# status-im/nim-blscurve

Hardware: AMD Instinct MI355X
Metric: BLS sig verifications/sec (batch) (higher is better)
Workload: dtype int64

## Files before the change

nim-blscurve_amd/csrc/kernels.hip:

```cpp
#include <hip/hip_runtime.h>

#include <algorithm>
#include <atomic>
#include <chrono>
#include <cstdio>
#include <cstdlib>
#include <cstring>
#include <mutex>
#include <string>
#include <unordered_map>
#include <vector>

#include "../../include/blscurve_mi355x.h"
#include "deser.hpp"
#include "h2c.hpp"
#include "pairing.hpp"
#include "vereach.hpp"
#include "aggsets.hpp"
#include "combsets.hpp"
#include "c12.hpp"
#include "teamvm.hpp"
#include "rowfp.hpp"
#include "rowvm.hpp"
#include "plan.hpp"
// ... 1519 lines not shown
    return g2_aff{fp2{ld_fp_int(w), ld_fp_int(w + FPW)}, fp2{ld_fp_int(w + 2 * FPW), ld_fp_int(w + 3 * FPW)}};
}
__device__ __forceinline__ g1_jac soa_ld_jac(const uint4* b, size_t stride, size_t i, const g1_jac*) { return soa_ld_g1(b, stride, i); }
__device__ __forceinline__ g2_jac soa_ld_jac(const uint4* b, size_t stride, size_t i, const g2_jac*) { return soa_ld_g2(b, stride, i); }
__device__ __forceinline__ void soa_st_jac(uint4* b, size_t stride, size_t i, const g1_jac& a) { soa_st_g1(b, stride, i, a); }
__device__ __forceinline__ void soa_st_jac(uint4* b, size_t stride, size_t i, const g2_jac& a) { soa_st_g2(b, stride, i, a); }
__device__ __forceinline__ g1_jac ld_jac_int(const uint32_t* w, const g1_jac*) { return ld_g1_int(w); }
__device__ __forceinline__ g2_jac ld_jac_int(const uint32_t* w, const g2_jac*) { return ld_g2_int(w); }
__device__ __forceinline__ void st_jac_int(uint32_t* w, const g1_jac& a) { st_g1_int(w, a); }
__device__ __forceinline__ void st_jac_int(uint32_t* w, const g2_jac& a) { st_g2_int(w, a); }
__device__ __forceinline__ void st_jac_blst(uint32_t* w, const g1_jac& a) { st_g1_blst(w, a); }
__device__ __forceinline__ void st_jac_blst(uint32_t* w, const g2_jac& a) { st_g2_blst(w, a); }
template <class F> struct fld;
template <> struct fld<fp> { static constexpr int W = FPW; static constexpr int AFFB = 96; };
template <> struct fld<fp2> { static constexpr int W = 2 * FPW; static constexpr int AFFB = 192; };
__device__ __forceinline__ g1_jac padd(const g1_jac& a, const g1_jac& b) { return jac_add_body(a, b); }
__device__ __forceinline__ g2_jac padd(const g2_jac& a, const g2_jac& b) { return jac_add(a, b); }

template <class F>
__global__ void __launch_bounds__(WAVE) k_pip_convert(const uint8_t* __restrict__ pts, uint32_t n, uint32_t* __restrict__ pts_int) {
    uint32_t i = blockIdx.x * WAVE + threadIdx.x;
    if (i >= n) return;
    aff<F> q = ld_aff_blst(reinterpret_cast<const uint32_t*>(pts + (size_t)i * fld<F>::AFFB), (const aff<F>*)nullptr);
    uint32_t* o = pts_int + (size_t)i * 2 * fld<F>::W;
    st_aff_int(o, q);
    o[FP_N] = aff_is_inf(q) ? 1u : 0u;
}
#if defined(__HIP_DEVICE_COMPILE__)
#include "../build/msm_asm.inc"
__device__ __forceinline__ uint32_t msm_bucket_asm(const uint32_t* pts, const uint32_t* srt, uint32_t cnt, uint4* buckets, uint32_t ostride16, uint32_t off16) {
    uint32_t flag;
    const uint64_t a = (uint64_t)(uintptr_t)srt;
    asm volatile(BLS_MSM_ASM_BODY : "=v"(flag) : "s"(pts), "v"((uint32_t)a), "v"((uint32_t)(a >> 32)), "v"(cnt), "s"(buckets), "s"(ostride16), "v"(off16) : BLS_MSM_ASM_CLOBBERS);
    return flag;
}
#endif
template <class F>
__global__ void __launch_bounds__(WAVE, sizeof(F) == sizeof(fp) ? 2 : 1) k_pip_bucket(const uint32_t* __restrict__ pts, const uint32_t* __restrict__ sorted, const uint32_t* __restrict__ offs,
                                                     const uint32_t* __restrict__ hist, const uint32_t* __restrict__ order, uint32_t n, uint32_t cbk,
                                                     uint32_t total, uint32_t g0, uint32_t gcount, uint4* __restrict__ buckets) {
    uint32_t t = blockIdx.x * WAVE + threadIdx.x;
    if (t >= gcount) return;
    uint32_t g = g0 + (order ? order[g0 + t] : t);
    uint32_t w = g >> cbk, cnt = hist[g], off = offs[g];
    const uint32_t* srt = sorted + (size_t)w * n + off;
#if defined(__HIP_DEVICE_COMPILE__)
    if constexpr (sizeof(F) == sizeof(fp)) {
        if (!msm_bucket_asm(pts, srt, cnt, buckets, total * 16u, g * 16u)) return;
    }
#endif
    xyzz<F> acc = xyzz_inf<F>();
    if (cnt) {
        uint32_t e = srt[0];
        const uint32_t* pw = pts + (size_t)(e & 0x7fffffffu) * (2 * fld<F>::W);
        aff<F> q = ld_aff_int(pw, (const aff<F>*)nullptr);
        if (e >> 31) q.y = f_neg(q.y);
        F one_or_zero = f_select(pw[FP_N] != 0, f_zero<F>(), f_one<F>());
        acc = xyzz<F>{q.x, q.y, one_or_zero, one_or_zero};
    }
    for (uint32_t j = 1; j < cnt; j++) {
        uint32_t e = srt[j];
        const uint32_t* pw = pts + (size_t)(e & 0x7fffffffu) * (2 * fld<F>::W);
        aff<F> q = ld_aff_int(pw, (const aff<F>*)nullptr);
        if (e >> 31) q.y = f_neg(q.y);
        acc = xyzz_add_aff_flag(acc, q, pw[FP_N] != 0);
    }
    soa_st_jac(buckets, total, g, jac_from_xyzz(acc));
}
template <class F>
__global__ void __launch_bounds__(WAVE) k_pip_segred(const uint4* __restrict__ buckets, uint32_t total, uint32_t cbk, uint32_t L, uint32_t nseg_total,
                                                     uint32_t t0, uint32_t tcount, uint4* __restrict__ segout) {
    uint32_t t = blockIdx.x * WAVE + threadIdx.x;
    if (t >= tcount) return;
    t += t0;
    uint32_t segs_per_win = (1u << cbk) / L;
    uint32_t w = t / segs_per_win, b0 = (t % segs_per_win) * L;
    jac<F> S = jac_inf<F>(), T = jac_inf<F>();
    for (uint32_t j = L; j-- > 0;) {
        jac<F> B = soa_ld_jac(buckets, total, ((size_t)w << cbk) | (b0 + j), (const jac<F>*)nullptr);
        S = padd(S, B);
        T = padd(T, S);
    }
    jac<F> acc = jac_inf<F>();
#pragma clang loop unroll(disable)
    for (int i = (int)cbk - 1; i >= 0; i--) {
        acc = jac_dbl(acc);
        if ((b0 >> i) & 1) acc = padd(acc, S);
    }
    acc = padd(acc, T);
    soa_st_jac(segout, nseg_total, t, acc);
}
template <int T>
struct team_quad_fp {
    uint32_t h;
    template <int J>
    __device__ __forceinline__ fp from(const fp& x) const {
        if (T == 4) return fp_quad_perm<J * 0x55>(x);
        return fp_quad_perm<(J ? 0xf5 : 0xa0)>(x);
    }
    __device__ __forceinline__ fp pick4(const fp& a0, const fp& a1, const fp& a2, const fp& a3) const {
        return fp_select((h & 1) != 0, fp_select((h & 2) != 0, a3, a1), fp_select((h & 2) != 0, a2, a0));
    }
    __device__ __forceinline__ void mul4(fp& r0, fp& r1, fp& r2, fp& r3, const fp& a0, const fp& b0, const fp& a1, const fp& b1, const fp& a2, const fp& b2, const fp& a3, const fp& b3) const {
        if (T == 4) {
            fp x = fp_mul(pick4(a0, a1, a2, a3), pick4(b0, b1, b2, b3));
            r0 = from<0>(x); r1 = from<1>(x); r2 = from<2>(x); r3 = from<3>(x);
        } else {
            const bool o = h != 0;
            fp x = fp_mul(fp_select(o, a1, a0), fp_select(o, b1, b0));
            fp y = fp_mul(fp_select(o, a3, a2), fp_select(o, b3, b2));
            r0 = from<0>(x); r1 = from<1>(x); r2 = from<0>(y); r3 = from<1>(y);
        }
    }
    __device__ __forceinline__ void mul3(fp& r0, fp& r1, fp& r2, const fp& a0, const fp& b0, const fp& a1, const fp& b1, const fp& a2, const fp& b2) const {
        fp r3;
        mul4(r0, r1, r2, r3, a0, b0, a1, b1, a2, b2, a2, b2);
    }
    __device__ __forceinline__ void sqr3(fp& r0, fp& r1, fp& r2, const fp& a0, const fp& a1, const fp& a2) const {
        if (T == 4) {
            fp x = fp_sqr(pick4(a0, a1, a2, a2));
            r0 = from<0>(x); r1 = from<1>(x); r2 = from<2>(x);
        } else {
            const bool o = h != 0;
            fp x = fp_sqr(fp_select(o, a1, a0));
            fp y = fp_sqr(a2);
            r0 = from<0>(x); r1 = from<1>(x); r2 = y;
        }
    }
    __device__ __forceinline__ void mul2(fp& r0, fp& r1, const fp& a0, const fp& b0, const fp& a1, const fp& b1) const {
        const bool o = (h & 1) != 0;
        fp x = fp_mul(fp_select(o, a1, a0), fp_select(o, b1, b0));
        if (T == 4) { r0 = fp_quad_perm<0xa0>(x); r1 = fp_quad_perm<0xf5>(x); }
        else { r0 = from<0>(x); r1 = from<1>(x); }
    }
    __device__ __forceinline__ void sqr2(fp& r0, fp& r1, const fp& a0, const fp& a1) const {
        const bool o = (h & 1) != 0;
        fp x = fp_sqr(fp_select(o, a1, a0));
        if (T == 4) { r0 = fp_quad_perm<0xa0>(x); r1 = fp_quad_perm<0xf5>(x); }
        else { r0 = from<0>(x); r1 = from<1>(x); }
    }
    __device__ __forceinline__ fp mul1(const fp& a, const fp& b) const { return fp_mul(a, b); }
};
template <int T>
__global__ void __launch_bounds__(WAVE) k_pip_segred_team(const uint4* __restrict__ buckets, uint32_t total, uint32_t cbk, uint32_t L, uint32_t nseg_total,
                                                          uint32_t t0, uint32_t tcount, uint4* __restrict__ segout) {
    uint32_t lane = blockIdx.x * WAVE + threadIdx.x, t = lane / T;
    if (t >= tcount) return;
    t += t0;
    const team_quad_fp<T> team{threadIdx.x & (T - 1)};
    uint32_t segs_per_win = (1u << cbk) / L;
    uint32_t w = t / segs_per_win, b0 = (t % segs_per_win) * L;
    g1_jac S = jac_inf<fp>(), Tt = jac_inf<fp>();
#pragma clang loop unroll(disable)
    for (uint32_t j = L; j-- > 0;) {
        g1_jac B = soa_ld_g1(buckets, total, ((size_t)w << cbk) | (b0 + j));
        S = jac_add_team(S, B, team);
        Tt = jac_add_team(Tt, S, team);
    }
    g1_jac acc = jac_inf<fp>();
#pragma clang loop unroll(disable)
    for (int i = (int)cbk - 1; i >= 0; i--) {
        acc = jac_dbl_team(acc, team);
        if ((b0 >> i) & 1) acc = jac_add_team(acc, S, team);
    }
    acc = jac_add_team(acc, Tt, team);
    if ((threadIdx.x & (T - 1)) == 0) soa_st_g1(segout, nseg_total, t, acc);
}
template <class F>
__global__ void __launch_bounds__(WAVE) k_pip_winpart(const uint4* __restrict__ segout, uint32_t nseg_total, uint32_t segs_per_win, uint32_t w0, uint32_t* __restrict__ part) {
    uint32_t w = w0 + blockIdx.x, sp = blockIdx.y, nsplit = gridDim.y;
    jac<F> acc = jac_inf<F>();
    for (uint32_t j = sp * WAVE + threadIdx.x; j < segs_per_win; j += WAVE * nsplit)
        acc = padd(acc, soa_ld_jac(segout, nseg_total, (size_t)w * segs_per_win + j, (const jac<F>*)nullptr));
    for (int d = 32; d >= 1; d >>= 1) {
        jac<F> o = shfl_down_struct(acc, d);
        acc = padd(acc, o);
    }
    if (threadIdx.x == 0) st_jac_int(part + ((size_t)w * nsplit + sp) * (3 * fld<F>::W), acc);
}
__device__ __forceinline__ fp fp_bcast(const fp& a, int src) {
    fp r;
#pragma unroll
    for (int i = 0; i < FP_N; i++) r.l[i] = __shfl(a.l[i], src, WAVE);
    return r;
}
struct team_wave_fp {
    __device__ __forceinline__ void mul3(fp& r0, fp& r1, fp& r2, const fp& a0, const fp& b0, const fp& a1, const fp& b1, const fp& a2, const fp& b2) const {
        const uint32_t l = threadIdx.x;
        fp r = fp_mul(fp_select(l == 0, a0, fp_select(l == 1, a1, a2)), fp_select(l == 0, b0, fp_select(l == 1, b1, b2)));
        r0 = fp_bcast(r, 0); r1 = fp_bcast(r, 1); r2 = fp_bcast(r, 2);
    }
    __device__ __forceinline__ void sqr3(fp& r0, fp& r1, fp& r2, const fp& a0, const fp& a1, const fp& a2) const {
        const uint32_t l = threadIdx.x;
        fp r = fp_sqr(fp_select(l == 0, a0, fp_select(l == 1, a1, a2)));
        r0 = fp_bcast(r, 0); r1 = fp_bcast(r, 1); r2 = fp_bcast(r, 2);
    }
    __device__ __forceinline__ fp mul1(const fp& a, const fp& b) const { return fp_mul(a, b); }
};
__device__ __forceinline__ g1_jac g1_dbl_coop(const g1_jac& p) { return jac_dbl_team(p, team_quad_fp<4>{threadIdx.x & 3u}); }
__device__ __forceinline__ g1_jac dbl_coop(const g1_jac& p) { return g1_dbl_coop(p); }
__device__ __forceinline__ g2_jac dbl_coop(const g2_jac& p) { return g2_dbl_coop(p, threadIdx.x & ~7u, threadIdx.x & 7u); }
__device__ __forceinline__ g1_jac bcast0(const g1_jac& a) { return g1_jac{fp_bcast(a.x, 0), fp_bcast(a.y, 0), fp_bcast(a.z, 0)}; }
__device__ __forceinline__ g2_jac bcast0(const g2_jac& a) {
    return g2_jac{fp2{fp_bcast(a.x.c0, 0), fp_bcast(a.x.c1, 0)}, fp2{fp_bcast(a.y.c0, 0), fp_bcast(a.y.c1, 0)}, fp2{fp_bcast(a.z.c0, 0), fp_bcast(a.z.c1, 0)}};
}
template <class F>
__global__ void __launch_bounds__(WAVE) k_pip_winsum(const uint32_t* __restrict__ part, uint32_t nsplit, pip_win W, uint32_t w0, uint32_t* __restrict__ winout) {
    uint32_t w = w0 + blockIdx.x;
    jac<F> acc = jac_inf<F>();
    for (uint32_t j = threadIdx.x; j < nsplit; j += WAVE) acc = padd(acc, ld_jac_int(part + ((size_t)w * nsplit + j) * (3 * fld<F>::W), (const jac<F>*)nullptr));
    int top = 32;
    while (top >= 1 && (uint32_t)top >= nsplit) top >>= 1;
    for (int d = top; d >= 1; d >>= 1) {
        jac<F> o = shfl_down_struct(acc, d);
        acc = padd(acc, o);
    }
    acc = bcast0(acc);
    uint32_t sh = pip_off(W, w);
#pragma clang loop unroll(disable)
    for (uint32_t i = 0; i < sh; i++) acc = dbl_coop(acc);
    if (threadIdx.x == 0) st_jac_int(winout + (size_t)w * (3 * fld<F>::W), acc);
}
__global__ void __launch_bounds__(1024) k_pip_rowtail(const uint32_t* __restrict__ part, uint32_t nsplit, pip_win W, uint32_t w0, uint32_t w1, const uint32_t* __restrict__ acc_in,
                                                      uint32_t* __restrict__ acc_out, uint32_t* __restrict__ out) {
    __shared__ uint32_t sums[64 * 48];
    const row_ctx C = row_ctx_make();
    const uint32_t wave = threadIdx.x >> 6, nwaves = blockDim.x >> 6, l16 = threadIdx.x & 15u;
    const bool row0 = (threadIdx.x & 63u) < 16u;
#pragma clang loop unroll(disable)
    for (uint32_t w = w0 + wave; w < w1; w += nwaves) {
        const uint32_t* base = part + (size_t)w * nsplit * (3 * FPW);
        row_g1 acc{row_load(base), row_load(base + FPW), row_load(base + 2 * FPW)};
#pragma clang loop unroll(disable)
        for (uint32_t j = 1; j < nsplit; j++) {
            const uint32_t* q = base + (size_t)j * (3 * FPW);
            acc = row_add(C, acc, row_g1{row_load(q), row_load(q + FPW), row_load(q + 2 * FPW)});
        }
        if (row0) {
            uint32_t* d = sums + (w - w0) * 48;
            d[l16] = (uint32_t)acc.x; d[16 + l16] = (uint32_t)acc.y; d[32 + l16] = (uint32_t)acc.z;
        }
    }
    __syncthreads();
    if (wave != 0) return;
    row_g1 acc;
    uint32_t w = w1;
    if (acc_in) {
        acc = row_g1{(rw)acc_in[l16], (rw)acc_in[16 + l16], (rw)acc_in[32 + l16]};
    } else {
        w--;
        const uint32_t* d = sums + (w - w0) * 48;
        acc = row_g1{(rw)d[l16], (rw)d[16 + l16], (rw)d[32 + l16]};
    }
#pragma clang loop unroll(disable)
    while (w > w0) {
        w--;
        const uint32_t sh = pip_off(W, w + 1) - pip_off(W, w);
#pragma clang loop unroll(disable)
        for (uint32_t i = 0; i < sh; i++) acc = row_dbl(C, acc);
        const uint32_t* d = sums + (w - w0) * 48;
        acc = row_add(C, acc, row_g1{(rw)d[l16], (rw)d[16 + l16], (rw)d[32 + l16]});
    }
    if (w0 == 0) {
        const g1_jac r{fp_reduce(row_to_fp(acc.x)), fp_reduce(row_to_fp(acc.y)), fp_reduce(row_to_fp(acc.z))};
        if (threadIdx.x == 0) st_jac_blst(out, r);
    } else if (row0) {
        acc_out[l16] = (uint32_t)acc.x; acc_out[16 + l16] = (uint32_t)acc.y; acc_out[32 + l16] = (uint32_t)acc.z;
    }
}
template <class F>
__global__ void __launch_bounds__(WAVE) k_pip_final(const uint32_t* __restrict__ winout, uint32_t nparts, uint32_t* __restrict__ out) {
    jac<F> acc = jac_inf<F>();
    for (uint32_t j = threadIdx.x; j < nparts; j += WAVE) acc = padd(acc, ld_jac_int(winout + (size_t)j * (3 * fld<F>::W), (const jac<F>*)nullptr));
    int top = 32;
    while (top >= 1 && (uint32_t)top >= nparts) top >>= 1;
    for (int d = top; d >= 1; d >>= 1) {
        jac<F> o = shfl_down_struct(acc, d);
        acc = padd(acc, o);
    }
    if (threadIdx.x == 0) st_jac_blst(out, acc);
}

__device__ __forceinline__ g1_jac ld_jac_blst(const uint32_t* w, const g1_jac*) { return ld_g1_blst(w); }
__device__ __forceinline__ g2_jac ld_jac_blst(const uint32_t* w, const g2_jac*) { return ld_g2_blst(w); }
template <class F>
__global__ void __launch_bounds__(WAVE) k_jac_sum_blst(const uint32_t* __restrict__ parts, uint32_t k, uint32_t stride, uint32_t* __restrict__ out) {
    jac<F> acc = jac_inf<F>();
    for (uint32_t j = threadIdx.x; j < k; j += WAVE) acc = padd(acc, ld_jac_blst(parts + (size_t)j * stride, (const jac<F>*)nullptr));
    int top = 32;
    while (top >= 1 && (uint32_t)top >= k) top >>= 1;
    for (int d = top; d >= 1; d >>= 1) {
        jac<F> o = shfl_down_struct(acc, d);
        acc = padd(acc, o);
    }
    if (threadIdx.x == 0) st_jac_blst(out, acc);
}

__global__ void __launch_bounds__(WAVE) k_sig_convert(const uint8_t* __restrict__ sets, uint32_t n, uint32_t* __restrict__ pts_int) {
    uint32_t i = blockIdx.x * WAVE + threadIdx.x;
    if (i >= n) return;
    g2_aff q = ld_g2a_blst(reinterpret_cast<const uint32_t*>(sets + (size_t)i * 320 + 128));
    uint32_t* o = pts_int + (size_t)i * 4 * FPW;
    st_fp_int(o, q.x.c0); st_fp_int(o + FPW, q.x.c1); st_fp_int(o + 2 * FPW, q.y.c0); st_fp_int(o + 3 * FPW, q.y.c1);
}
__global__ void __launch_bounds__(WAVE) k_sig_consts(uint32_t c, uint32_t total, uint32_t* __restrict__ out) {
    uint32_t g = blockIdx.x * WAVE + threadIdx.x;
    if (g >= total) return;
    uint64_t sc = (uint64_t)(g & ((1u << c) - 1u)) << (c * (g >> c));
    g1_aff ng{fp_from_const(k::G1_X), fp_from_const(k::G1_NEG_Y)};
    st_g1_int(out + (size_t)g * G1W, jac_mul_u64(ng, sc));
}
__global__ void __launch_bounds__(WAVE) k_sig_bucket(const uint32_t* __restrict__ pts, const uint32_t* __restrict__ sorted, const uint32_t* __restrict__ offs,
                                                     const uint32_t* __restrict__ hist, uint32_t n, uint32_t c, uint32_t lshift, uint32_t total,
                                                     const uint32_t* __restrict__ consts, uint4* __restrict__ H, uint4* __restrict__ P, size_t stride, size_t base) {
    uint32_t t = blockIdx.x * WAVE + threadIdx.x;
    uint32_t L = 1u << lshift, g = t >> lshift, s = t & (L - 1);
    xyzz<fp2> part = xyzz_inf<fp2>();
    if (g < total) {
        uint32_t w = g >> c, cnt = hist[g], off = offs[g];
        const uint32_t* srt = sorted + (size_t)w * n + off;
        for (uint32_t j = s; j < cnt; j += L) {
            const uint32_t* pw = pts + (size_t)srt[j] * (4 * FPW);
            g2_aff q{fp2{ld_fp_int(pw), ld_fp_int(pw + FPW)}, fp2{ld_fp_int(pw + 2 * FPW), ld_fp_int(pw + 3 * FPW)}};
            part = xyzz_add_aff(part, q);
        }
    }
    g2_jac acc = jac_from_xyzz(part);
    for (uint32_t d = L >> 1; d >= 1; d >>= 1) {
        g2_jac o = shfl_down_struct(acc, (int)d);
        acc = jac_add(acc, o);
    }
    if (g < total && s == 0) {
        soa_st_g2(H, stride, base + g, acc);
        soa_st_g1(P, stride, base + g, ld_g1_int(consts + (size_t)g * G1W));
    }
}
__global__ void __launch_bounds__(WAVE) k_sig_fold(const uint4* __restrict__ H, size_t stride, uint32_t n, uint32_t nwin, uint32_t c, uint32_t* __restrict__ agg_out) {
    __shared__ uint32_t wsum[32 * G2W];
    uint32_t w = threadIdx.x;
    if (w < nwin) {
        g2_jac S = jac_inf<fp2>(), T = jac_inf<fp2>();
        for (uint32_t d = (1u << c) - 1; d >= 1; d--) {
            S = jac_add(S, soa_ld_g2(H, stride, (size_t)n + ((w << c) | d)));
            T = jac_add(T, S);
        }
        st_g2_int(wsum + (size_t)w * G2W, T);
    }
    __syncthreads();
    if (threadIdx.x == 0) {
        g2_jac acc = ld_g2_int(wsum + (size_t)(nwin - 1) * G2W);
        for (uint32_t j = nwin - 1; j-- > 0;) {
            for (uint32_t i = 0; i < c; i++) acc = jac_dbl(acc);
            acc = jac_add(acc, ld_g2_int(wsum + (size_t)j * G2W));
        }
        st_g2_blst(agg_out, acc);
    }
}

__global__ void __launch_bounds__(WAVE) k_deser(const uint8_t* __restrict__ pks, const uint8_t* __restrict__ msgs, const uint8_t* __restrict__ sigs,
                                                uint32_t n, uint32_t dflags, uint8_t* __restrict__ sets, uint8_t* __restrict__ status,
                                                uint32_t* __restrict__ flags) {
    uint32_t i = blockIdx.x * WAVE + threadIdx.x;
    if (i >= n) return;
    g1_aff pk;
    g2_aff sg;
    const size_t pkb = (dflags & DESER_F_PK_UNCOMPRESSED) ? 96 : 48, sgb = (dflags & DESER_F_SIG_UNCOMPRESSED) ? 192 : 96;
    uint8_t st = deserialize_tuple(pk, sg, pks + (size_t)i * pkb, sigs + (size_t)i * sgb, dflags);
    status[i] = st;
    if (st != DESER_OK) atomicOr(flags + 2, 1u);
    uint32_t* o = reinterpret_cast<uint32_t*>(sets + (size_t)i * 320);
    bool ok = st == DESER_OK;
    pk = g1_aff{fp_select(ok, pk.x, fp_zero()), fp_select(ok, pk.y, fp_zero())};
    sg = g2_aff{fp2_select(ok, sg.x, fp2_zero()), fp2_select(ok, sg.y, fp2_zero())};
    st_fp_blst(o, pk.x); st_fp_blst(o + 12, pk.y);
    const uint8_t* m = msgs + (size_t)i * 32;
    for (int j = 0; j < 8; j++) o[24 + j] = (uint32_t)m[4 * j] | ((uint32_t)m[4 * j + 1] << 8) | ((uint32_t)m[4 * j + 2] << 16) | ((uint32_t)m[4 * j + 3] << 24);
    st_fp_blst(o + 32, sg.x.c0); st_fp_blst(o + 44, sg.x.c1); st_fp_blst(o + 56, sg.y.c0); st_fp_blst(o + 68, sg.y.c1);
}

__global__ void k_finish_affine(const uint32_t* __restrict__ p1, const uint32_t* __restrict__ p2, uint32_t* __restrict__ out_pk, uint32_t* __restrict__ out_sig) {
    if (threadIdx.x != 0 || blockIdx.x != 0) return;
    g1_jac a = ld_g1_blst(p1);
    if (jac_is_inf(a)) {
        for (int i = 0; i < 24; i++) out_pk[i] = 0;
    } else {
        fp zi = fp_inv(a.z), zi2 = fp_sqr(zi);
        st_fp_blst(out_pk, fp_mul(a.x, zi2));
        st_fp_blst(out_pk + 12, fp_mul(a.y, fp_mul(zi2, zi)));
    }
    g2_jac b{fp2{ld_fp_blst(p2), ld_fp_blst(p2 + 12)}, fp2{ld_fp_blst(p2 + 24), ld_fp_blst(p2 + 36)}, fp2{ld_fp_blst(p2 + 48), ld_fp_blst(p2 + 60)}};
    if (jac_is_inf(b)) {
        for (int i = 0; i < 48; i++) out_sig[i] = 0;
    } else {
        fp2 zi = fp2_inv(b.z), zi2 = fp2_sqr(zi);
        fp2 x = fp2_mul(b.x, zi2), y = fp2_mul(b.y, fp2_mul(zi2, zi));
        st_fp_blst(out_sig, x.c0); st_fp_blst(out_sig + 12, x.c1); st_fp_blst(out_sig + 24, y.c0); st_fp_blst(out_sig + 36, y.c1);
    }
}

__global__ void __launch_bounds__(WAVE) k_hash_var(const uint8_t* __restrict__ msgs, const uint32_t* __restrict__ offs, uint32_t n, dst_t dst,
                                                   uint4* __restrict__ H, size_t stride) {
    uint32_t i = blockIdx.x * blockDim.x + threadIdx.x;
    if (i >= n) return;
    g2_jac h = hash_to_g2(msgs + offs[i], offs[i + 1] - offs[i], dst.b, dst.len);
    soa_st_g2(H, stride, i, h);
}
__global__ void __launch_bounds__(WAVE) k_aggv_records(const uint8_t* __restrict__ msgs, uint32_t n, uint8_t* __restrict__ recs) {
    uint32_t i = blockIdx.x * blockDim.x + threadIdx.x;
    if (i >= n) return;
    for (int j = 0; j < 32; j++) recs[(size_t)i * 320 + 96 + j] = msgs[(size_t)i * 32 + j];
}
__global__ void __launch_bounds__(WAVE) k_aggv_setup(const uint8_t* __restrict__ pks, uint32_t n, int with_sig, const uint32_t* __restrict__ sig, uint4* __restrict__ H,
                                                     uint4* __restrict__ P, size_t stride, uint32_t* __restrict__ flags) {
    uint32_t i = blockIdx.x * blockDim.x + threadIdx.x;
    if (i < n) {
        g1_aff pk = ld_g1a_blst(reinterpret_cast<const uint32_t*>(pks + (size_t)i * 96));
        if (aff_is_inf(pk)) atomicOr(flags, 1u);
        soa_st_g1(P, stride, i, jac_from_aff(pk));
    } else if (i == n && with_sig) {
        soa_st_g1(P, stride, n, g1_jac{fp_from_const(k::G1_X), fp_from_const(k::G1_NEG_Y), fp_one()});
        soa_st_g2(H, stride, n, jac_from_aff(ld_g2a_blst(sig)));
    }
}

__global__ void __launch_bounds__(WAVE) k_each_setup(const uint8_t* __restrict__ sets, uint32_t m, uint4* __restrict__ H, uint4* __restrict__ P, size_t stride) {
    uint32_t i = blockIdx.x * blockDim.x + threadIdx.x;
    if (i >= m) return;
    const uint32_t* w = reinterpret_cast<const uint32_t*>(sets + (size_t)i * 320);
    soa_st_g1(P, stride, i, jac_from_aff(ld_g1a_blst(w)));
    soa_st_g1(P, stride, (size_t)m + i, g1_jac{fp_from_const(k::G1_X), fp_from_const(k::G1_NEG_Y), fp_one()});
    soa_st_g2(H, stride, (size_t)m + i, jac_from_aff(ld_g2a_blst(w + 32)));
}
__global__ void __launch_bounds__(WAVE) __attribute__((amdgpu_waves_per_eu(1, 1)))
k_each_tail(const uint4* __restrict__ lines, size_t stride, uint32_t m, const uint8_t* __restrict__ sets, uint8_t* __restrict__ verdicts, uint32_t* __restrict__ gt) {
    uint32_t i = blockIdx.x * blockDim.x + threadIdx.x;
    if (i >= m) return;
    const auto line_of = [&](int s, size_t j) {
        const uint4* b = lines + (size_t)s * 24 * stride;
        return line_t{soa_ld2(b, stride, 0, j), soa_ld2(b, stride, 2, j), soa_ld2(b, stride, 4, j)};
    };
    const bool pk_inf = aff_is_inf(ld_g1a_blst(reinterpret_cast<const uint32_t*>(sets + (size_t)i * 320)));
    const vereach_out o = vereach_set([&](int s) { return line_of(s, i); }, [&](int s) { return line_of(s, (size_t)m + i); }, pk_inf);
    verdicts[i] = o.ok ? 1 : 0;
    if (gt) {
        uint32_t* g = gt + (size_t)i * 144;
        const fp2* c[6] = {&o.value.c0.a0, &o.value.c0.a1, &o.value.c0.a2, &o.value.c1.a0, &o.value.c1.a1, &o.value.c1.a2};
        for (int t = 0; t < 6; t++) {
            st_fp_blst(g + 24 * t, c[t]->c0);
            st_fp_blst(g + 24 * t + 12, c[t]->c1);
        }
    }
}
constexpr uint32_t EACH_WORK_STATE = N_LINES * F12W, EACH_WORK_GT = EACH_WORK_STATE + 144, EACH_WORK_V = EACH_WORK_GT + 144, EACH_WORK_WORDS = EACH_WORK_V + 16;
template <bool ROWS>
__device__ __forceinline__ void each_engine_body(const uint4* __restrict__ lines, size_t stride, uint32_t m, const uint8_t* __restrict__ sets,
                                                 uint8_t* __restrict__ verdicts, uint32_t* __restrict__ gt, uint32_t* __restrict__ work) {
    uint32_t* W = work + (size_t)blockIdx.x * EACH_WORK_WORDS;
    for (uint32_t i = blockIdx.x; i < m; i += gridDim.x) {
        if (threadIdx.x < WAVE) {
            for (uint32_t s = threadIdx.x; s < (uint32_t)N_LINES; s += WAVE) {
                const uint4* b = lines + (size_t)s * 24 * stride;
                const line_t la{soa_ld2(b, stride, 0, i), soa_ld2(b, stride, 2, i), soa_ld2(b, stride, 4, i)};
                const size_t j = (size_t)m + i;
                const line_t lb{soa_ld2(b, stride, 0, j), soa_ld2(b, stride, 2, j), soa_ld2(b, stride, 4, j)};
                st_fp12_int(W + (size_t)s * F12W, fp12_reduce(fp12_mul_by_line(fp12_from_line(la), lb)));
            }
        }
        __syncthreads();
        tail_body<ROWS>(W, W + EACH_WORK_STATE, 1, 3, W + EACH_WORK_GT, W + EACH_WORK_V, 144, 0);
        __syncthreads();
        if (threadIdx.x == 0) {
            const bool pk_inf = aff_is_inf(ld_g1a_blst(reinterpret_cast<const uint32_t*>(sets + (size_t)i * 320)));
            verdicts[i] = (W[EACH_WORK_V] == 1u && !pk_inf) ? 1 : 0;
        }
        if (gt && threadIdx.x < 144) gt[(size_t)i * 144 + threadIdx.x] = W[EACH_WORK_GT + threadIdx.x];
        __syncthreads();
    }
}
__global__ void __launch_bounds__(TAIL_THREADS) k_each_engine(const uint4* __restrict__ lines, size_t stride, uint32_t m, const uint8_t* __restrict__ sets,
                                                              uint8_t* __restrict__ verdicts, uint32_t* __restrict__ gt, uint32_t* __restrict__ work) {
    each_engine_body<false>(lines, stride, m, sets, verdicts, gt, work);
}
__global__ void __launch_bounds__(K_TAIL_THREADS) k_each_engine_rows(const uint4* __restrict__ lines, size_t stride, uint32_t m, const uint8_t* __restrict__ sets,
                                                                     uint8_t* __restrict__ verdicts, uint32_t* __restrict__ gt, uint32_t* __restrict__ work) {
    each_engine_body<true>(lines, stride, m, sets, verdicts, gt, work);
}

__global__ void __launch_bounds__(WAVE, 2) k_aggsets_l0(const uint4* __restrict__ items, uint32_t n_items, const uint8_t* __restrict__ keys, size_t n_table,
                                                        const uint32_t* __restrict__ idx, uint32_t* __restrict__ part, uint32_t* __restrict__ seg_bad) {
    uint32_t i = blockIdx.x * blockDim.x + threadIdx.x;
    if (i >= n_items) return;
    const uint4 it = items[i];
    const g1_jac acc = aggsets_l0_item(it.x, it.y, idx, n_table,
                                       [&](size_t t) { return ld_g1a_blst(reinterpret_cast<const uint32_t*>(keys + t * 96)); },
                                       [&]() { atomicOr(seg_bad + it.w, 1u); });
    st_g1_int(part + (size_t)it.z * G1W, acc);
}
__global__ void __launch_bounds__(WAVE, 2) k_aggsets_ln(const uint4* __restrict__ items, uint32_t n_items, uint32_t* __restrict__ part) {
    uint32_t i = blockIdx.x * blockDim.x + threadIdx.x;
    if (i >= n_items) return;
    const uint4 it = items[i];
    const g1_jac acc = aggsets_ln_item(it.x, it.y, [&](uint32_t j) { return ld_g1_int(part + (size_t)j * G1W); });
    st_g1_int(part + (size_t)it.z * G1W, acc);
}
__global__ void __launch_bounds__(WAVE) k_aggsets_finish(const uint32_t* __restrict__ final_of, uint32_t k, const uint32_t* __restrict__ part,
                                                         const uint32_t* __restrict__ seg_bad, const uint32_t* __restrict__ msgs, const uint32_t* __restrict__ sigs,
                                                         uint32_t* __restrict__ records, uint8_t* __restrict__ status) {
    uint32_t s = blockIdx.x * blockDim.x + threadIdx.x;
    if (s >= k) return;
    const uint32_t f = final_of[s];
    const bool empty = f == 0xffffffffu;
    const aggsets_end e = aggsets_finish_item(empty, seg_bad[s] != 0, empty ? jac_inf<fp>() : ld_g1_int(part + (size_t)f * G1W));
    uint32_t* r = records + (size_t)s * 80;
    for (int i = 0; i < 24; i++) r[i] = e.pk[i];
    for (int i = 0; i < 8; i++) r[24 + i] = msgs[(size_t)s * 8 + i];
    for (int i = 0; i < 48; i++) r[32 + i] = sigs[(size_t)s * 48 + i];
    status[s] = e.status;
}

__global__ void __launch_bounds__(256) k_combsets_gather(const uint32_t* __restrict__ sets, size_t n_sets, const uint32_t* __restrict__ idx, uint32_t n,
                                                         uint32_t* __restrict__ out) {
    const size_t t = (size_t)blockIdx.x * 256 + threadIdx.x, pos = t / 80, w = t % 80;
    if (pos >= n) return;
    const size_t at = idx[pos];
    out[t] = at < n_sets ? sets[at * 80 + w] : 0u;
}
__global__ void __launch_bounds__(WAVE) k_combsets_scalars(const uint32_t* __restrict__ seg_first, const uint32_t* __restrict__ seg_len, uint32_t k,
                                                           const uint8_t* __restrict__ rnds, uint32_t lane_max, uint64_t* __restrict__ s) {
    uint32_t g = blockIdx.x * blockDim.x + threadIdx.x;
    if (g >= k) return;
    const uint32_t len = seg_len[g];
    uint64_t* o = s + seg_first[g];
    if (len == 1) o[0] = 0;
    if (len < 2 || len > lane_max) return;
    uint8_t rnd[32];
    for (int i = 0; i < 32; i++) rnd[i] = rnds[(size_t)g * 32 + i];
    combsets_chain(rnd, len, [&](size_t j, uint64_t v) { o[j] = v; });
}
__global__ void __launch_bounds__(WAVE) k_combsets_g2mul(const uint32_t* __restrict__ recs, uint32_t n, const uint64_t* __restrict__ s, uint4* __restrict__ tab,
                                                         size_t tcap, uint32_t* __restrict__ out) {
    uint32_t i = blockIdx.x * blockDim.x + threadIdx.x;
    if (i >= n) return;
    const g2_aff q = ld_g2a_blst(recs + (size_t)i * 80 + 32);
    const g2_jac r = combsets_mul_item(q, s[i], [&](int e, const g2_jac& t) { soa_st_g2(tab, 8 * tcap, (size_t)e * tcap + i, t); },
                                       [&](int e) { return soa_ld_g2(tab, 8 * tcap, (size_t)e * tcap + i); });
    st_g2_int(out + (size_t)i * G2W, r);
}
__global__ void __launch_bounds__(WAVE, 2) k_combsets_g1_l0(const uint4* __restrict__ items, uint32_t n_items, const uint4* __restrict__ P, size_t stride,
                                                            const uint32_t* __restrict__ recs, const uint32_t* __restrict__ idx, size_t n_sets,
                                                            const uint32_t* __restrict__ seg_first, uint32_t* __restrict__ part, uint32_t* __restrict__ seg_flags) {
    uint32_t i = blockIdx.x * blockDim.x + threadIdx.x;
    if (i >= n_items) return;
    const uint4 it = items[i];
    const uint32_t fl = combsets_check_item(it.x, it.y, seg_first[it.w], [&](uint32_t pos) { return idx && idx[pos] >= n_sets; },
                                            [&](uint32_t pos) { return recs + (size_t)pos * 80; });
    if (fl) atomicOr(seg_flags + it.w, fl);
    st_g1_int(part + (size_t)it.z * G1W, aggsets_ln_item(it.x, it.y, [&](uint32_t j) { return soa_ld_g1(P, stride, j); }));
}
__global__ void __launch_bounds__(WAVE) k_combsets_g2_sum(const uint4* __restrict__ items, uint32_t n_items, const uint32_t* __restrict__ src, uint32_t* __restrict__ dst) {
    uint32_t i = blockIdx.x * blockDim.x + threadIdx.x;
    if (i >= n_items) return;
    const uint4 it = items[i];
    st_g2_int(dst + (size_t)it.z * G2W, combsets_sum_item<fp2>(it.x, it.y, [&](uint32_t j) { return ld_g2_int(src + (size_t)j * G2W); }));
}
__global__ void __launch_bounds__(WAVE) k_combsets_finish(const uint32_t* __restrict__ final_of, const uint32_t* __restrict__ seg_first,
                                                          const uint32_t* __restrict__ seg_len, uint32_t k, const uint32_t* __restrict__ part1,
                                                          const uint32_t* __restrict__ part2, const uint32_t* __restrict__ seg_flags, const uint32_t* __restrict__ recs,
                                                          const uint32_t* __restrict__ idx, size_t n_sets, uint32_t* __restrict__ records, uint8_t* __restrict__ status) {
    uint32_t g = blockIdx.x * blockDim.x + threadIdx.x;
    if (g >= k) return;
    const uint32_t f = final_of[g], len = seg_len[g], first = seg_first[g];
    const bool sums = len >= 2 && f != 0xffffffffu, have_first = len >= 1 && !(idx && idx[first] >= n_sets);
    const combsets_end e = combsets_finish_item(len, seg_flags[g], sums ? ld_g1_int(part1 + (size_t)f * G1W) : jac_inf<fp>(),
                                                sums ? ld_g2_int(part2 + (size_t)f * G2W) : jac_inf<fp2>(), have_first ? recs + (size_t)first * 80 : nullptr);
    uint32_t* r = records + (size_t)g * 80;
    for (int i = 0; i < 80; i++) r[i] = e.rec[i];
    status[g] = e.status;
}

BLS_HD bool sk_load_check(uint32_t (&kk)[8], const uint8_t* sk) {
    uint32_t any = 0, borrow = 0;
#pragma unroll
    for (int j = 0; j < 8; j++) {
        kk[j] = (uint32_t)sk[4 * j] | ((uint32_t)sk[4 * j + 1] << 8) | ((uint32_t)sk[4 * j + 2] << 16) | ((uint32_t)sk[4 * j + 3] << 24);
        any |= kk[j];
        uint64_t d = (uint64_t)kk[j] - k::R_ORDER[j] - borrow;
        borrow = (uint32_t)(d >> 63);
    }
    return any != 0 && borrow != 0;
}
__global__ void __launch_bounds__(WAVE) k_sign_pk(const uint8_t* __restrict__ sks, const uint8_t* __restrict__ msgs, uint32_t n, uint8_t* __restrict__ sets,
                                                  uint8_t* __restrict__ status, uint32_t* __restrict__ flags) {
    uint32_t i = blockIdx.x * WAVE + threadIdx.x;
    if (i >= n) return;
    uint32_t kk[8];
    bool ok = sk_load_check(kk, sks + (size_t)i * 32);
    status[i] = ok ? 0 : 1;
    if (!ok) atomicOr(flags + 2, 1u);
    uint32_t* o = reinterpret_cast<uint32_t*>(sets + (size_t)i * 320);
    g1_aff g{fp_from_const(k::G1_X), fp_from_const(k::G1_Y)};
    g1_jac a = jac_mul_256(g, kk);
    fp zi = fp_inv(a.z), zi2 = fp_sqr(zi);
    fp x = fp_select(ok, fp_mul(a.x, zi2), fp_zero()), y = fp_select(ok, fp_mul(a.y, fp_mul(zi2, zi)), fp_zero());
    st_fp_blst(o, x); st_fp_blst(o + 12, y);
    const uint8_t* m = msgs + (size_t)i * 32;
    for (int j = 0; j < 8; j++) o[24 + j] = (uint32_t)m[4 * j] | ((uint32_t)m[4 * j + 1] << 8) | ((uint32_t)m[4 * j + 2] << 16) | ((uint32_t)m[4 * j + 3] << 24);
}
__global__ void __launch_bounds__(WAVE) k_sign_sig(const uint8_t* __restrict__ sks, const uint8_t* __restrict__ msgs, uint32_t n, dst_t dst,
                                                   uint8_t* __restrict__ sets) {
    uint32_t i = blockIdx.x * WAVE + threadIdx.x;
    if (i >= n) return;
    uint32_t kk[8];
    bool ok = sk_load_check(kk, sks + (size_t)i * 32);
    uint8_t msg[32];
    for (int j = 0; j < 32; j++) msg[j] = msgs[(size_t)i * 32 + j];
    g2_jac h = hash_to_g2(msg, 32, dst.b, dst.len);
    g2_jac a = jac_mul_256_jac(h, kk);
    fp2 zi = fp2_inv(a.z), zi2 = fp2_sqr(zi);
    fp2 x = fp2_select(ok, fp2_mul(a.x, zi2), fp2_zero()), y = fp2_select(ok, fp2_mul(a.y, fp2_mul(zi2, zi)), fp2_zero());
    uint32_t* o = reinterpret_cast<uint32_t*>(sets + (size_t)i * 320) + 32;
    st_fp_blst(o, x.c0); st_fp_blst(o + 12, x.c1); st_fp_blst(o + 24, y.c0); st_fp_blst(o + 36, y.c1);
}

// ... 103 lines not shown
```

Baseline: 6.074 million.

## Use hand-written assembly for G2 bucket accumulation with a fallback on edge cases

Replaces the compiled G2 bucket-accumulation loop in k_sig_bucket with an inline assembly body included from a generated file. The body returns an XYZZ partial sum plus a flag, and when the flag is set the code discards the result and reruns the original C++ loop. The signature conversion kernel now writes an infinity flag next to each point so the assembly can see that case. The goal is tighter register use and scheduling in the hot field arithmetic. The cost is a build dependency on a generated .inc file and the risk that hand-written assembly diverges from the reference path.

Result: no change. 6.040 million (-0.6%).

```diff
diff --git a/nim-blscurve_amd/csrc/kernels.hip b/nim-blscurve_amd/csrc/kernels.hip
--- a/nim-blscurve_amd/csrc/kernels.hip
+++ b/nim-blscurve_amd/csrc/kernels.hip
@@ -1845,6 +1845,7 @@
     g2_aff q = ld_g2a_blst(reinterpret_cast<const uint32_t*>(sets + (size_t)i * 320 + 128));
     uint32_t* o = pts_int + (size_t)i * 4 * FPW;
     st_fp_int(o, q.x.c0); st_fp_int(o + FPW, q.x.c1); st_fp_int(o + 2 * FPW, q.y.c0); st_fp_int(o + 3 * FPW, q.y.c1);
+    o[FP_N] = aff_is_inf(q) ? 1u : 0u;
 }
 __global__ void __launch_bounds__(WAVE) k_sig_consts(uint32_t c, uint32_t total, uint32_t* __restrict__ out) {
     uint32_t g = blockIdx.x * WAVE + threadIdx.x;
@@ -1853,15 +1854,44 @@
     g1_aff ng{fp_from_const(k::G1_X), fp_from_const(k::G1_NEG_Y)};
     st_g1_int(out + (size_t)g * G1W, jac_mul_u64(ng, sc));
 }
+#if defined(__HIP_DEVICE_COMPILE__) && !defined(BLS_SIGBUCKET_NOASM)
+#include "../build/g2bucket_asm.inc"
+typedef uint32_t bls_u32x16 __attribute__((ext_vector_type(16)));
+__device__ __forceinline__ uint32_t g2bucket_asm(const uint32_t* pts, const uint32_t* first, uint32_t entries, uint32_t step_bytes, xyzz<fp2>& part) {
+    uint32_t flag;
+    bls_u32x16 o0, o1, o2, o3, o4, o5, o6;
+    const uint64_t a = (uint64_t)(uintptr_t)first;
+    asm volatile(BLS_G2BUCKET_ASM_BODY : "=v"(flag), BLS_G2BUCKET_ASM_OUTS(o0, o1, o2, o3, o4, o5, o6)
+                 : "s"(pts), "v"((uint32_t)a), "v"((uint32_t)(a >> 32)), "v"(entries), "s"(step_bytes) : BLS_G2BUCKET_ASM_CLOBBERS);
+    const bls_u32x16 o[7] = {o0, o1, o2, o3, o4, o5, o6};
+    fp* f[8] = {&part.x.c0, &part.x.c1, &part.y.c0, &part.y.c1, &part.zz.c0, &part.zz.c1, &part.zzz.c0, &part.zzz.c1};
+#pragma unroll
+    for (int k = 0; k < 8; k++) {
+#pragma unroll
+        for (int i = 0; i < FP_N; i++) f[k]->l[i] = o[(FP_N * k + i) / 16][(FP_N * k + i) % 16];
+    }
+    return flag;
+}
+#endif
 __global__ void __launch_bounds__(WAVE) k_sig_bucket(const uint32_t* __restrict__ pts, const uint32_t* __restrict__ sorted, const uint32_t* __restrict__ offs,
                                                      const uint32_t* __restrict__ hist, uint32_t n, uint32_t c, uint32_t lshift, uint32_t total,
                                                      const uint32_t* __restrict__ consts, uint4* __restrict__ H, uint4* __restrict__ P, size_t stride, size_t base) {
     uint32_t t = blockIdx.x * WAVE + threadIdx.x;
     uint32_t L = 1u << lshift, g = t >> lshift, s = t & (L - 1);
     xyzz<fp2> part = xyzz_inf<fp2>();
+    uint32_t cnt = 0;
+    const uint32_t* srt = sorted;
     if (g < total) {
-        uint32_t w = g >> c, cnt = hist[g], off = offs[g];
-        const uint32_t* srt = sorted + (size_t)w * n + off;
+        uint32_t w = g >> c, off = offs[g];
+        cnt = hist[g];
+        srt = sorted + (size_t)w * n + off;
+    }
+    bool redo = true;
+#if defined(__HIP_DEVICE_COMPILE__) && !defined(BLS_SIGBUCKET_NOASM)
+    redo = g2bucket_asm(pts, srt + s, cnt > s ? (cnt - s + L - 1) >> lshift : 0u, 4u << lshift, part) != 0;
+    if (redo) part = xyzz_inf<fp2>();
+#endif
+    if (redo) {
         for (uint32_t j = s; j < cnt; j += L) {
             const uint32_t* pw = pts + (size_t)srt[j] * (4 * FPW);
             g2_aff q{fp2{ld_fp_int(pw), ld_fp_int(pw + FPW)}, fp2{ld_fp_int(pw + 2 * FPW), ld_fp_int(pw + 3 * FPW)}};
```
